# MakisChristou/fhestring

Measured on AMD Instinct MI355X. Metric: PBS/sec and ms/op for contains() on N-char FheString, higher is better.
Workload: dtype f64

## Files before the change

bindings/fhestring_hip.rs:

```rust
#![allow(non_camel_case_types, dead_code)]
use std::os::raw::{c_char, c_int, c_void};

pub const FHS_LWE_N: c_int = 742;
pub const FHS_POLY_N: c_int = 2048;
pub const FHS_BIG_CT: c_int = 2049;
pub const FHS_SMALL_CT: c_int = 743;
pub const FHS_BLOCKS_PER_CHAR: c_int = 4;
pub const FHS_CHAR_WORDS: usize = 8196;
pub const FHS_BSK_WORDS: usize = 6078464;
pub const FHS_KSK_WORDS: usize = 7608320;
pub const FHS_MAX_FIND_LENGTH: c_int = 255;
pub const FHS_MAX_REPETITIONS: c_int = 16;
pub const FHS_OK: c_int = 0;
pub const FHS_ERR_ARG: c_int = -1;
pub const FHS_ERR_HIP: c_int = -2;
pub const FHS_ERR_STATE: c_int = -3;
pub const FHS_ERR_LIMIT: c_int = -4;
pub const FHS_ARITH_EXACT_NTT: c_int = 0;
pub const FHS_ARITH_F64_FFT: c_int = 1;
pub const FHS_ARITH_F64_FFT_MB2: c_int = 2;
pub const FHS_ARITH_EXACT_NTT_MB2: c_int = 3;
pub const FHS_BSK_MB2_WORDS: usize = 9117696;
pub const FHS_MODE_AS_WRITTEN: c_int = 0;
pub const FHS_MODE_FUSED: c_int = 1;
pub const FHS_DIST_ID_BYTES: usize = 128;
pub const FHS_TRANSPORT_NONE: c_int = 0;
pub const FHS_TRANSPORT_RCCL: c_int = 1;
pub const FHS_TRANSPORT_HOST: c_int = 2;
pub const FHS_NOISE_BUDGET_SUM_C2: c_int = 64;
pub const FHS_DOM_SEEDED_STR: c_int = 4;
pub const FHS_DOM_SEEDED_BSK: c_int = 5;
pub const FHS_DOM_SEEDED_KSK: c_int = 6;
pub const FHS_SEED_WORDS: usize = 8;
pub const FHS_CSTR_BODY_WORDS: usize = 4;
pub const FHS_CBSK_BODY_WORDS: usize = 3039232;
pub const FHS_CKSK_BODY_WORDS: usize = 10240;
pub const FHS_CKEY_FILE_BYTES: usize = 24395872;
pub const FHS_PACK_BASE_LOG: c_int = 16;
pub const FHS_PACK_LEVELS: c_int = 3;
pub const FHS_PACK_TREE_LEVELS: c_int = 11;
pub const FHS_PACK_GROUP: c_int = 2048;
pub const FHS_PACK_KEY_WORDS: usize = 135168;
pub const FHS_PACK_KEY_FILE_BYTES: usize = 1081408;
// ... 147 lines not shown
    pub fn fhs_dist_str_compare(c: *mut fhs_ctx, a: *const fhs_char_t, na: usize, b: *const fhs_char_t, nb: usize, cmp: c_int, out: *mut fhs_char_t) -> c_int;
    pub fn fhs_dist_level_parallel(ctx: *mut fhs_ctx, on: c_int) -> c_int;
    pub fn fhs_dist_config(ctx: *mut fhs_ctx, rank: c_int, world: c_int) -> c_int;
    pub fn fhs_flush_plan(ctx: *mut fhs_ctx, n_levels: *mut u64, max_level_width: *mut u64) -> c_int;
    pub fn fhs_flush_level_exec(ctx: *mut fhs_ctx, level: u64, d_slice: *mut u64, width: *mut u64, cap: *mut u64) -> c_int;
    pub fn fhs_flush_level_commit(ctx: *mut fhs_ctx, level: u64, d_all: *const u64) -> c_int;
    pub fn fhs_stream_sync(ctx: *mut fhs_ctx) -> c_int;
    pub fn fhs_debug_capture_pbs_inputs(ctx: *mut fhs_ctx, max_rows_per_level: usize) -> c_int;
    pub fn fhs_debug_capture_live(ctx: *mut fhs_ctx, on: c_int) -> c_int;
    pub fn fhs_debug_capture_read(ctx: *mut fhs_ctx, rows: *mut u64, recs: *mut fhs_capture_rec, cap: usize, n: *mut usize) -> c_int;
    pub fn fhs_debug_plan_trace(ctx: *mut fhs_ctx, on: c_int) -> c_int;
    pub fn fhs_debug_plan_read(ctx: *mut fhs_ctx, out: *mut u64, cap: usize, n: *mut usize) -> c_int;
    pub fn fhs_debug_char_terms(ctx: *mut fhs_ctx, h: fhs_char_t, out: *mut u64, cap: usize, n: *mut usize) -> c_int;
    pub fn fhs_debug_lut_poly(lut_id: c_int, out: *mut u64) -> c_int;
    pub fn fhs_debug_live_resources(out: *mut u64) -> c_int;
    pub fn fhs_get_stats(ctx: *mut fhs_ctx, out: *mut fhs_stats) -> c_int;
    pub fn fhs_char_sum_c2(ctx: *mut fhs_ctx, h: fhs_char_t, out: *mut u64) -> c_int;
    pub fn fhs_char_set_noise(ctx: *mut fhs_ctx, h: fhs_char_t, sum_c2: u64) -> c_int;
    pub fn fhs_trivial_value(ctx: *mut fhs_ctx, h: fhs_char_t, is_trivial: *mut c_int, value: *mut u8) -> c_int;
    pub fn fhs_level_widths(ctx: *mut fhs_ctx, out: *mut u32, cap: usize, n: *mut usize) -> c_int;
    pub fn fhs_launch_groups(ctx: *mut fhs_ctx, out: *mut u32, cap: usize, n: *mut usize) -> c_int;
    pub fn fhs_reset_stats(ctx: *mut fhs_ctx) -> c_int;
    pub fn fhs_client_create(out: *mut *mut fhs_client) -> c_int;
    pub fn fhs_client_create_insecure_seeded(seed: u64, out: *mut *mut fhs_client) -> c_int;
    pub fn fhs_chacha20_block(key: *const u32, counter: u32, nonce: *const u32, out: *mut u32);
    pub fn fhs_chacha20_stream(key: *const u32, counter: u32, nonce: *const u32, out: *mut u64, n: usize);
    pub fn fhs_client_destroy(ck: *mut fhs_client);
    pub fn fhs_client_bsk(ck: *const fhs_client) -> *const u64;
    pub fn fhs_client_ksk(ck: *const fhs_client) -> *const u64;
    pub fn fhs_client_bsk_mb2(ck: *mut fhs_client) -> *const u64;
// ... 53 lines not shown
```

fhestring_amd/api.py:

```python
import ctypes as C

import numpy as np

from . import cabi
from ._lib import FhsError, lib, check_single_hip_runtime

_K = dict(cabi.parse_header()["consts"])
BIG_CT = _K["FHS_BIG_CT"]
SMALL_CT = _K["FHS_SMALL_CT"]
POLY_N = _K["FHS_POLY_N"]
PACK_GROUP = _K["FHS_PACK_GROUP"]
PACK_KEY_WORDS = _K["FHS_PACK_KEY_WORDS"]


def _ptr(a):
    return a.ctypes.data_as(C.c_void_p)


class Context:

    def __init__(self, device_id=0, planner=False):
        self._L = lib()
        if not planner:
            check_single_hip_runtime()
# ... 97 lines not shown
        return out

    def pbs_batch_shifted(self, cts, lut_idx, luts, shifts):
        cts = np.ascontiguousarray(cts, np.uint64).reshape(-1, BIG_CT)
        luts = np.ascontiguousarray(luts, np.uint64).reshape(-1, POLY_N)
        lut_idx = np.ascontiguousarray(lut_idx, np.uint32)
        B = cts.shape[0]
        shifts = np.ascontiguousarray(shifts, np.uint32).reshape(B, -1)
        out = np.zeros((B, shifts.shape[1], BIG_CT), np.uint64)
        self._check(self._L.fhs_pbs_batch_shifted(self._h, _ptr(cts), _ptr(lut_idx), _ptr(luts), luts.shape[0],
                                                  _ptr(shifts), shifts.shape[1], _ptr(out), B))
        return out

    def set_rotation_sharing(self, on=True):
        self._check(self._L.fhs_set_rotation_sharing(self._h, int(bool(on))))

    def keyswitch_modswitch_batch(self, cts):
        cts = np.ascontiguousarray(cts, np.uint64).reshape(-1, BIG_CT)
        B = cts.shape[0]
        out = np.zeros((B, SMALL_CT), np.uint32)
        self._check(self._L.fhs_keyswitch_modswitch_batch(self._h, _ptr(cts), _ptr(out), B))
        return out

    def pbs_batch_device(self, d_in, d_lut_idx, d_luts, d_out, B, stream=0):
        self._check(self._L.fhs_pbs_batch_device(self._h, C.c_void_p(d_in), C.c_void_p(d_lut_idx),
                                                 C.c_void_p(d_luts), C.c_void_p(d_out), int(B),
                                                 C.c_void_p(stream)))

    def kernel_timing(self, reset=False):
        br, ks = C.c_double(), C.c_double()
# ... 1046 lines not shown
```

fhestring_amd/csrc/capi_core.cpp:

```cpp
#include <algorithm>
#include <new>

#include "capi_internal.h"
#include "keyfile.h"
#include "luts.h"
#include "seeded_kernels.h"

extern "C" {

int fhs_ctx_create(int device_id, fhs_ctx **out) {
    if (!out) return FHS_ERR_ARG;
    *out = nullptr;
    fhs_ctx *c = new (std::nothrow) fhs_ctx();
    if (!c) return FHS_ERR_STATE;
    int rc = c->eng.ctx.init(device_id);
    if (rc) {
        *out = c;
        return rc;
    }
    *out = c;
    return FHS_OK;
}

int fhs_ctx_create_planner(fhs_ctx **out) {
// ... 187 lines not shown
    const fhs::Bid *b = ctx->eng.char_blocks(h);
    for (int k = 0; k < 4; k++) ctx->eng.describe_block(b[k], v);
    *n = v.size();
    if (!out) return FHS_OK;
    if (cap < v.size()) return ctx->eng.ctx.fail(FHS_ERR_ARG, "fhs_debug_char_terms: buffer too small");
    std::copy(v.begin(), v.end(), out);
    return FHS_OK;
}

int fhs_debug_live_resources(uint64_t out[5]) {
    if (!out) return FHS_ERR_ARG;
    fhs::live_resources(out);
    return FHS_OK;
}

int fhs_debug_lut_poly(int lut_id, uint64_t *out) {
    if (!out || lut_id < 0 || lut_id >= fhs::LUT_COUNT) return FHS_ERR_ARG;
    fhs::make_lut_poly(lut_id, out);
    return FHS_OK;
}

int fhs_debug_capture_read(fhs_ctx *ctx, uint64_t *rows, fhs_capture_rec *recs, size_t cap, size_t *n) {
    if (!ctx || !n) return FHS_ERR_ARG;
    auto &e = ctx->eng;
    static_assert(sizeof(fhs_capture_rec) == sizeof(fhs::Engine::CaptureRec), "record layout");
    const size_t have = e.capture_recs.size();
    if (!rows || !recs) { *n = have; return FHS_OK; }
    const size_t k = std::min(cap, have);
    std::copy(e.capture_rows.begin(), e.capture_rows.begin() + k * fhs::BIG_CT, rows);
    std::copy(e.capture_recs.begin(), e.capture_recs.begin() + k,
// ... 33 lines not shown
```

fhestring_amd/csrc/context.cpp:

```cpp
#include "context.h"
#include "pack_kernels.h"
#include "seeded_kernels.h"
#include "../../include/fhestring_hip.h"

#include <algorithm>
#include <cstdlib>
#include <utility>

namespace fhs {

namespace {
constexpr size_t KSK_BYTES = (size_t)BIG_N * KS_LEVEL * SMALL_CT * sizeof(uint64_t);
constexpr size_t BSK_BYTES = (size_t)LWE_N * 4 * POLY_N * sizeof(uint64_t);
}

#define HIP_TRY(expr, what)                                \
    do {                                                   \
        hipError_t e__ = (expr);                           \
        if (e__ != hipSuccess) return hip_fail(e__, what); \
    } while (0)

Event KernelTimer::get() {
    if (pool.empty()) return Event();
    Event e = std::move(pool.back());
// ... 60 lines not shown
            if (end == q) break;
            mask.push_back((uint32_t)w);
            bits += __builtin_popcount((uint32_t)w);
            q = *end == ',' ? end + 1 : end;
            if (*end != ',') break;
        }
        if (mask.empty() || bits == 0 || bits > cus) return fail(-1, "FHS_STREAM_CU_MASK: expected hex words selecting 1.." + std::to_string(cus) + " CUs");
        HIP_TRY(stream.create(mask.data(), (uint32_t)mask.size()), "hipExtStreamCreateWithCUMask");
        cus = bits;
    } else {
        HIP_TRY(stream.create(), "hipStreamCreate");
    }
    wg_slots = 4 * cus;
    launch_chunk[FHS_ARITH_F64_FFT_MB2] = (size_t)wg_slots;
    launch_chunk[FHS_ARITH_F64_FFT] = (size_t)wg_slots;
    HIP_TRY(d_work_counter.reserve_exact(64), "hipMalloc counter");
    return 0;
}

Context::~Context() {
    if (stream) (void)hipStreamSynchronize(stream);
    dist.shutdown();
    timer.resolve();
}

int Context::load_server_key(const uint64_t *bsk, const uint64_t *ksk) {
    if (!bsk || !ksk) return fail(-1, "null key pointer");
    HIP_TRY(hipSetDevice(device), "hipSetDevice");
    DevBuf d_ksk;
    HIP_TRY(d_ksk.reserve_exact(KSK_BYTES), "hipMalloc ksk staging");
    hipError_t e = hipMemcpy(d_ksk.ptr, ksk, KSK_BYTES, hipMemcpyHostToDevice);
// ... 108 lines not shown
}

int Context::keyswitch(const uint64_t *d_in, size_t B, hipStream_t s) {
    if (dig_buf.cap < ks_digits_bytes((int)B)) {
        HIP_TRY(hipStreamSynchronize(s), "sync");
        HIP_TRY(dig_buf.reserve(ks_digits_bytes((int)B)), "hipMalloc digits");
    }
    timer.begin(1, B, s);
    hipError_t e = launch_keyswitch_mfma(d_in, d_ksk_planes.as<int8_t>(), dig_buf.as<int8_t>(), ks_buf.as<uint64_t>(), (int)B, s,
                                         wg_slots / 4);
    timer.end(s);
    if (e != hipSuccess) return hip_fail(e, "keyswitch launch");
    return 0;
}

int Context::set_arithmetic(int mode) {
    if (mode < 0 || mode >= N_ARITH) return fail(-1, "unknown arithmetic mode");
    if (is_f64_fft(mode) && key_loaded && !d_bsk_fft)
        if (int rc = build_fft_key()) return rc;
    if (mode == FHS_ARITH_F64_FFT_MB2 && key_loaded && !d_bsk_mb)
        return fail(-3, "the two-bits-per-product arithmetic needs the pair key in the Fourier domain: call "
                        "fhs_load_multibit_key while arithmetic 1 (f64 FFT) is selected, then fhs_set_arithmetic 2");
    if (mode == FHS_ARITH_EXACT_NTT_MB2 && key_loaded && !d_bsk_ntt_mb)
        return fail(-3, "the exact two-bits-per-product arithmetic needs the pair key converted to residues: call "
                        "fhs_load_multibit_key while the EXACT arithmetic (fhs_set_arithmetic 0) is selected, then "
                        "fhs_set_arithmetic 3");
    arith = mode;
    return 0;
}

// ... 39 lines not shown
    HIP_TRY(prepare_device_for_packing(), "kernel attributes");
    return 0;
}

int Context::blind_rotate(const uint64_t *d_ks, const uint32_t *d_lut_idx, const uint64_t *d_luts, uint64_t *d_out,
                          uint64_t *const *d_out_ptrs, size_t B, hipStream_t s, uint64_t *const *d_body_ptrs) {
    hipError_t e = hipSuccess;
    const bool four = arith == FHS_ARITH_F64_FFT && B <= (size_t)fft4_max_batch;
    if (arith == FHS_ARITH_F64_FFT_MB2 && !d_bsk_mb) return fail(-3, "pair key not loaded (fhs_load_multibit_key)");
    if (arith == FHS_ARITH_EXACT_NTT_MB2 && !d_bsk_ntt_mb)
        return fail(-3, "pair key not loaded in the exact arithmetic (fhs_load_multibit_key)");
    if (arith == FHS_ARITH_F64_FFT && !d_bsk_fft) return fail(-3, "Fourier-domain key not loaded");
    timer.begin(four ? 2 : 0, B, s);
    const size_t chunk = (launch_chunk[arith] && !four) ? launch_chunk[arith] : B;
    uint32_t n_launches = 0;
    for (size_t off = 0, n = 0; off < B && e == hipSuccess; off += n) {
        n = std::min(chunk, B - off);
        if (B - off - n < chunk / 4) n = B - off;
        n_launches++;
        const uint64_t *ks = d_ks + off * SMALL_CT;
        const uint32_t *li = d_lut_idx + off;
        uint64_t *out = d_out ? d_out + off * BIG_CT : nullptr;
        uint64_t *const *outp = d_out_ptrs ? d_out_ptrs + off : nullptr;
        uint64_t *const *bodyp = d_body_ptrs ? d_body_ptrs + off : nullptr;
        if (arith == FHS_ARITH_EXACT_NTT_MB2) {
            BlindRotateNttMb2Params p{};
            p.ks = ks; p.lut_idx = li; p.luts = d_luts;
            p.bsk_ntt_mb = d_bsk_ntt_mb.as<double>(); p.tw = tw; p.crt_c = crt_c; p.mono = d_ntt_mono;
            p.out = out; p.out_ptrs = outp; p.body_ptrs = bodyp; p.B = (int)n;
            e = launch_blind_rotate_ntt_mb2(p, s);
        } else if (arith == FHS_ARITH_F64_FFT_MB2) {
            BlindRotateMb2Params p{};
            p.ks = ks; p.lut_idx = li; p.luts = d_luts;
            p.bsk_mb = d_bsk_mb.as<double>();
            p.lanetab = ft.lanetab; p.mono = ft.mono; p.r16 = ft.r16;
            p.work_counter = d_work_counter.as<uint32_t>();
            p.slots = wg_slots;
            p.out = out; p.out_ptrs = outp; p.body_ptrs = bodyp; p.B = (int)n;
            e = launch_blind_rotate_mb2(p, s);
        } else if (arith == FHS_ARITH_F64_FFT) {
            BlindRotateFftParams p{};
            p.ks = ks; p.lut_idx = li; p.luts = d_luts;
            p.bsk_fft = d_bsk_fft.as<double>();
            p.lanetab = ft.lanetab; p.weff = ft.weff;
            p.work_counter = d_work_counter.as<uint32_t>();
            p.slots = wg_slots;
            p.out = out; p.out_ptrs = outp; p.body_ptrs = bodyp; p.B = (int)n;
            e = four ? launch_blind_rotate_fft4(p, s) : launch_blind_rotate_fft(p, s);
        } else {
            BlindRotateParams p{};
            p.ks = ks; p.lut_idx = li; p.luts = d_luts;
            p.bsk_ntt = d_bsk_ntt.as<double>(); p.tw = tw; p.crt_c = crt_c;
            p.out = out; p.out_ptrs = outp; p.body_ptrs = bodyp; p.B = (int)n;
            e = launch_blind_rotate(p, s);
        }
    }
    timer.end(s, n_launches);
    if (e != hipSuccess) return hip_fail(e, "blind_rotate launch");
    return 0;
}

int Context::pbs_batch_device(const uint64_t *d_in, const uint32_t *d_lut_idx, const uint64_t *d_luts,
                              uint64_t *d_out, size_t B, hipStream_t s) {
// ... 117 lines not shown
```

fhestring_amd/csrc/context.h:

```cpp
#pragma once
#include <hip/hip_runtime.h>

#include <cstdint>
#include <string>
#include <vector>

#include "../../include/fhestring_hip.h"
#include "dist.h"
#include "fft_tables.h"
#include "hip_owners.h"
#include "ntt_tables.h"
#include "pbs_kernels.h"

namespace fhs {

constexpr int N_ARITH = 4;
constexpr bool is_f64_fft(int arith) { return arith == FHS_ARITH_F64_FFT || arith == FHS_ARITH_F64_FFT_MB2; }

struct FftTablePtrs {
    const double *lanetab = nullptr;
    const double *weff = nullptr;
    const double *mono = nullptr;
    const double *r16 = nullptr;
};
// ... 20 lines not shown
    std::string err;
    bool key_loaded = false;

    DevBuf d_ksk_planes;
    DevBuf d_bsk_ntt;
    DevBuf d_tables;
    NttTables tw{};
    double crt_c = 0;

    int arith = FHS_ARITH_EXACT_NTT;
    DevBuf d_bsk_fft;
    DevBuf d_bsk_std;
    DevBuf d_fft_tables;
    FftTablePtrs ft;
    DevBuf d_work_counter;
    int wg_slots = 1024;
    DevBuf d_bsk_mb;
    DevBuf d_bsk_ntt_mb;
    const double *d_ntt_mono = nullptr;
    DevBuf d_pack_key_ntt;
    int load_packing_key(const uint64_t *key);
    int load_multibit_key(const uint64_t *bsk_mb2);
    int fft4_max_batch = 512;
    size_t launch_chunk[N_ARITH] = {};
    int set_arithmetic(int mode);
    int keyswitch(const uint64_t *d_in, size_t B, hipStream_t s);
    int blind_rotate(const uint64_t *d_ks, const uint32_t *d_lut_idx, const uint64_t *d_luts, uint64_t *d_out,
                     uint64_t *const *d_out_ptrs, size_t B, hipStream_t s, uint64_t *const *d_body_ptrs = nullptr);

    Dist dist;
    DevBuf xchg_send, xchg_recv;

    DevBuf dig_buf;
    DevBuf ks_buf, ms_buf, in_buf, out_buf, lutidx_buf, luts_buf, tab_buf;
    DevBuf pack_ws[2], pack_tab, pack_out;
    KernelTimer timer;

    int init(int device_id);
    ~Context();
    int fail(int code, const std::string &msg) { err = msg; return code; }
    int hip_fail(hipError_t e, const char *what);
// ... 18 lines not shown
```

fhestring_amd/csrc/engine.cpp:

```cpp
#include "engine.h"
#include "../../include/fhestring_hip.h"

#include <algorithm>
#include <cstdio>
#include <cstdlib>
#include <cstring>
#include <map>

namespace fhs {

int Engine::on_key_loaded() {
    if (!d_luts_) {
        std::vector<uint64_t> host((size_t)LUT_COUNT * POLY_N);
        for (int id = 0; id < LUT_COUNT; id++) make_lut_poly(id, host.data() + (size_t)id * POLY_N);
        hipError_t e = d_luts_.reserve_exact(host.size() * 8);
        if (e != hipSuccess) return ctx.hip_fail(e, "hipMalloc luts");
        e = hipMemcpy(d_luts_.ptr, host.data(), host.size() * 8, hipMemcpyHostToDevice);
        if (e != hipSuccess) return ctx.hip_fail(e, "copy luts");
    }
    return 0;
}

Engine::~Engine() {
    if (!planner && ctx.stream) (void)hipStreamSynchronize(ctx.stream);
// ... 714 lines not shown
        CaptureRec r = l.recs[first + i];
        r.level = level;
        capture_recs.push_back(r);
    }
    return 0;
}

int Engine::launch_rows(const GroupView &v, size_t lo, size_t cnt, uint64_t *dense_out, const TickLevel *levels,
                        size_t n_levels, size_t first_level) {
    const uint8_t *dp = tick_buf_.as<uint8_t>();
    const LinDesc *d_desc = reinterpret_cast<const LinDesc *>(dp);
    const LinTerm *d_terms = reinterpret_cast<const LinTerm *>(dp + v.off_terms);
    const uint32_t *d_lut = reinterpret_cast<const uint32_t *>(dp + v.off_lut);
    uint64_t *const *d_out = reinterpret_cast<uint64_t *const *>(dp + v.off_out);
    uint64_t *const *d_body = reinterpret_cast<uint64_t *const *>(dp + v.off_body);
    hipError_t e = launch_lincomb(d_desc + lo, d_terms, batch_in_.as<uint64_t>(), (int)cnt, ctx.stream);
    if (e != hipSuccess) return ctx.hip_fail(e, "lincomb launch");
    size_t row0 = 0;
    for (size_t j = 0; j < n_levels && capture_max_rows; j++) {
        const TickLevel &l = levels[j];
        const size_t w = l.descs.size(), a = std::max(lo, row0), b = std::min(lo + cnt, row0 + w);
        if (l.recs.size() == w && a < b)
            if (int rc = sample_capture(l, a - row0, b - a, a - lo, (uint32_t)(first_level + j))) return rc;
        row0 += w;
    }
    if (int rc = ctx.keyswitch(batch_in_.as<uint64_t>(), cnt, ctx.stream)) return rc;
    return ctx.blind_rotate(ctx.ks_buf.as<uint64_t>(), d_lut + lo, d_luts_.as<uint64_t>(), dense_out, dense_out ? nullptr : d_out + lo, cnt,
                            ctx.stream, v.n_ext && !dense_out ? d_body + lo : nullptr);
}

int Engine::scatter_rows(const uint64_t *d_all, uint64_t *const *d_out, size_t width) {
    hipError_t e = launch_scatter_blocks(d_all, d_out, (int)width, ctx.stream);
    return e == hipSuccess ? 0 : ctx.hip_fail(e, "scatter launch");
}

void Engine::trace_group(const std::vector<TickLevel> &levels, size_t width) {
    for (auto &l : levels) {
        for (size_t k = 0; k < l.descs.size(); k++) {
            const LinDesc &d = l.descs[k];
            trace_.insert(trace_.end(), {TR_ROW, (uint64_t)(uintptr_t)l.out[k], l.lut[k], d.konst_body >> DELTA_LOG, d.n_terms});
            for (uint32_t t = 0; t < d.n_terms; t++) {
// ... 177 lines not shown
```

fhestring_amd/csrc/ks_kernels.hip:

```cpp
#include <cstdlib>

#include "pbs_kernels.h"

namespace fhs {

namespace {
typedef int v4i __attribute__((ext_vector_type(4)));
typedef int v16i __attribute__((ext_vector_type(16)));

constexpr int KS_K = BIG_N * KS_LEVEL;
constexpr int KS_STEPS = KS_K / 32;
constexpr int KS_COL_TILES = 24;
constexpr int KS_PLANES = 8;

__device__ __forceinline__ size_t frag_off(int r, int k) {
    return ((size_t)(k >> 5) * 64 + ((k >> 4) & 1) * 32 + r) * 16 + (k & 15);
}
}

__global__ __launch_bounds__(256) void ks_digits_kernel(const uint64_t *__restrict__ in, int8_t *__restrict__ dig, int B) {
    const int ct = blockIdx.x;
    int8_t *dst = dig + (size_t)(ct >> 5) * KS_STEPS * 1024;
    const int r = ct & 31;
    for (int i = threadIdx.x; i < BIG_N; i += 256) {
// ... 45 lines not shown
                    d[l] = x;
                }
            }
#pragma unroll
            for (int l = 0; l < KS_LEVEL; l++) {
                const int p = pos + l;
                if (p >= 0 && p < 16) w[p >> 2] |= (uint32_t)(uint8_t)(int8_t)d[l] << (8 * (p & 3));
            }
        }
        v4i o;
        o.x = (int)w[0]; o.y = (int)w[1]; o.z = (int)w[2]; o.w = (int)w[3];
        dst[(size_t)ks * 64] = o;
    }
}

__global__ __launch_bounds__(256) void ksk_to_planes_kernel(const uint64_t *__restrict__ ksk, int8_t *__restrict__ planes) {
    const int k = blockIdx.x;
    for (int j = threadIdx.x; j < KS_COL_TILES * 32; j += 256) {
        uint64_t w = j < SMALL_CT ? ksk[(size_t)k * SMALL_CT + j] : 0;
        const size_t off = (size_t)(j >> 5) * KS_STEPS * 1024 + frag_off(j & 31, k);
#pragma unroll
        for (int b = 0; b < KS_PLANES; b++) {
            const int8_t s = (int8_t)(w & 0xff);
            w = (w - (uint64_t)(int64_t)s) >> 8;
            planes[(size_t)b * KS_COL_TILES * KS_STEPS * 1024 + off] = s;
        }
    }
}

__global__ __launch_bounds__(256) void keyswitch_mfma_kernel(const int8_t *__restrict__ dig, const int8_t *__restrict__ planes,
// ... 147 lines not shown
}

hipError_t prepare_device_for_keyswitch() {
    return hipFuncSetAttribute(reinterpret_cast<const void *>(keyswitch_mfma2_kernel),
                               hipFuncAttributeMaxDynamicSharedMemorySize, KS2_LDS_BYTES);
}

size_t ks_planes_bytes() { return (size_t)KS_PLANES * KS_COL_TILES * KS_STEPS * 1024; }
size_t ks_digits_bytes(int B) { return (size_t)((B + 255) / 256) * 8 * KS_STEPS * 1024; }

hipError_t launch_ksk_to_planes(const uint64_t *d_ksk, int8_t *d_planes, hipStream_t s) {
    hipLaunchKernelGGL(ksk_to_planes_kernel, dim3(KS_K), dim3(256), 0, s, d_ksk, d_planes);
    return hipGetLastError();
}

hipError_t launch_keyswitch_mfma(const uint64_t *d_in, const int8_t *d_planes, int8_t *d_dig, uint64_t *d_ks_out, int B,
                                 hipStream_t s, int n_cus) {
    if (B <= 0) return hipSuccess;
    const int tiles = (B + 31) / 32;
    static const int old_below = [] { const char *v = std::getenv("FHS_KS_OLD_BELOW"); return v ? std::atoi(v) : KS2_MIN_BATCH; }();
    const bool wide = B >= old_below;
    if (wide)
        hipLaunchKernelGGL(ks_digits_tile_kernel, dim3(((B + KS2_GROUP - 1) / KS2_GROUP) * (KS2_GROUP / 32), KS_DIG_CHUNKS),
                           dim3(256), 0, s, d_in, d_dig, B);
    else
        hipLaunchKernelGGL(ks_digits_kernel, dim3(((tiles + 3) / 4) * 128), dim3(256), 0, s, d_in, d_dig, B);
    hipError_t e = hipGetLastError();
    if (e != hipSuccess) return e;
    if (wide) {
        const int n_groups = (B + KS2_GROUP - 1) / KS2_GROUP;
        const int tiles2 = KS_COL_TILES * n_groups, slots = n_cus > 0 ? n_cus : 256;
        int full = tiles2 / slots * slots, rem = tiles2 - full, slices = 1;
        if (rem > 0)
            for (int c : {8, 4, 2})
                if (rem * c <= slots) { slices = c; break; }
        if (slices == 1) { full = tiles2; rem = 0; }
        else {
            const size_t row0 = (size_t)(full / 8 / 3) * KS2_GROUP;
            if (row0 < (size_t)B) {
                e = hipMemsetAsync(d_ks_out + row0 * SMALL_CT, 0, ((size_t)B - row0) * SMALL_CT * 8, s);
                if (e != hipSuccess) return e;
            }
        }
        hipLaunchKernelGGL(keyswitch_mfma2_kernel, dim3(full + rem * slices), dim3(256), KS2_LDS_BYTES, s, d_dig, d_planes,
                           d_in, d_ks_out, B, n_groups, full, rem > 0 ? rem : 1, slices);
        return hipGetLastError();
    }
    int splits = 1;
    const int tgroups = (tiles + 3) / 4;
    while (splits < 16 && tgroups * KS_COL_TILES * splits < 256) splits *= 2;
    if (splits > 1) {
        e = hipMemsetAsync(d_ks_out, 0, (size_t)B * SMALL_CT * 8, s);
        if (e != hipSuccess) return e;
    }
    hipLaunchKernelGGL(keyswitch_mfma_kernel, dim3(tgroups, KS_COL_TILES, splits), dim3(256), 0, s, d_dig, d_planes,
                       d_in, d_ks_out, B, KS_STEPS / splits);
    return hipGetLastError();
}

}
```

fhestring_amd/csrc/pbs_kernels.h:

```cpp
#pragma once
#include <hip/hip_runtime.h>
#include <cstddef>
#include <cstdint>

namespace fhs {

constexpr int LWE_N = 742;
constexpr int POLY_N = 2048;
constexpr int BIG_N = 2048;
constexpr int BIG_CT = 2049;
constexpr int SMALL_CT = 743;
constexpr int KS_LEVEL = 5;
constexpr int KS_BASE_LOG = 3;
constexpr int DELTA_LOG = 59;
constexpr int BSK_QUANT_BITS = 6;

constexpr uint64_t NTT_P0 = 140737488273409ull;
constexpr uint64_t NTT_P1 = 140737488252929ull;
constexpr uint64_t NTT_PSI0 = 124135596386681ull;
constexpr uint64_t NTT_PSI1 = 116052249937262ull;

struct NttTables {
    const double *fwd_uni;
    const double *fwd_lane;
// ... 62 lines not shown
struct LinDesc {
    uint32_t first_term;
    uint32_t n_terms;
    uint64_t konst_body;
};
struct LinTerm {
    const uint64_t *src;
    int64_t coef;
};

size_t blind_rotate_lds_bytes();
hipError_t prepare_device_for_kernels();
hipError_t read_device_ntt_consts(double *fwd_uni , double *inv_uni , double *crt);
hipError_t launch_blind_rotate(const BlindRotateParams &p, hipStream_t s);
hipError_t launch_blind_rotate_fft(const BlindRotateFftParams &p, hipStream_t s);
hipError_t launch_blind_rotate_fft4(const BlindRotateFftParams &p, hipStream_t s);
hipError_t launch_bsk_to_fft(const uint64_t *d_bsk_std, double *d_out, const double *d_lanetab, hipStream_t s,
                             int n_polys = LWE_N * 4);
hipError_t launch_blind_rotate_mb2(const BlindRotateMb2Params &p, hipStream_t s);
hipError_t launch_blind_rotate_ntt_mb2(const BlindRotateNttMb2Params &p, hipStream_t s);
hipError_t prepare_device_for_ntt_mb2();
hipError_t prepare_device_for_fft4();
hipError_t prepare_device_for_keyswitch();
void fft_uniform_consts(double *w_re, double *w_im, double *u_re, double *u_im);
size_t ks_planes_bytes();
size_t ks_digits_bytes(int B);
hipError_t launch_ksk_to_planes(const uint64_t *d_ksk, int8_t *d_planes, hipStream_t s);
hipError_t launch_keyswitch_mfma(const uint64_t *d_in , const int8_t *d_planes, int8_t *d_dig ,
                                 uint64_t *d_ks_out , int B, hipStream_t s, int n_cus = 256);
hipError_t launch_modswitch(const uint64_t *d_ks, uint32_t *d_ms , int B, hipStream_t s);
hipError_t launch_lincomb(const LinDesc *d_desc, const LinTerm *d_terms, uint64_t *d_out ,
                          int n, hipStream_t s);
hipError_t launch_scatter_blocks(const uint64_t *d_in, uint64_t *const *d_dst, int n, hipStream_t s);
hipError_t launch_gather_rows(const uint64_t *const *d_src, uint64_t *d_out, int n, hipStream_t s);
struct ExtractDesc {
    const uint64_t *lead;
    const uint64_t *body;
    uint64_t *out;
    uint32_t K, pad;
};
hipError_t launch_extract_shift(const ExtractDesc *d_desc, int n, hipStream_t s);

}
```

include/fhestring_hip.h:

```cpp
#ifndef FHESTRING_HIP_H
#define FHESTRING_HIP_H

#include <stddef.h>
#include <stdint.h>

#ifdef __cplusplus
extern "C" {
#endif

#define FHS_LWE_N 742
#define FHS_POLY_N 2048
#define FHS_BIG_CT 2049
#define FHS_SMALL_CT 743
#define FHS_BLOCKS_PER_CHAR 4
#define FHS_CHAR_WORDS (4 * 2049)
#define FHS_BSK_WORDS ((size_t)742 * 4 * 2048)
#define FHS_KSK_WORDS ((size_t)2048 * 5 * 743)
#define FHS_MAX_FIND_LENGTH 255
#define FHS_MAX_REPETITIONS 16

#define FHS_OK 0
#define FHS_ERR_ARG (-1)
#define FHS_ERR_HIP (-2)
#define FHS_ERR_STATE (-3)
// ... 151 lines not shown
    uint32_t lut;
    uint32_t n_terms;
    int64_t sum_c2;
    int32_t konst;
    uint32_t width;
} fhs_capture_rec;
int fhs_debug_capture_pbs_inputs(fhs_ctx *ctx, size_t max_rows_per_level);
int fhs_debug_capture_live(fhs_ctx *ctx, int on);
int fhs_debug_capture_read(fhs_ctx *ctx, uint64_t *rows, fhs_capture_rec *recs, size_t cap, size_t *n);

int fhs_debug_plan_trace(fhs_ctx *ctx, int on);
int fhs_debug_plan_read(fhs_ctx *ctx, uint64_t *out, size_t cap, size_t *n);
int fhs_debug_char_terms(fhs_ctx *ctx, fhs_char_t h, uint64_t *out, size_t cap, size_t *n);
int fhs_debug_lut_poly(int lut_id, uint64_t *out);
int fhs_debug_live_resources(uint64_t out[5]);

typedef struct {
    uint64_t pbs_executed;
    uint64_t pbs_folded;
    uint64_t levels;
    uint64_t max_level_width;
    uint64_t blocks_live;
    uint64_t max_input_sum_c2;
    uint64_t pbs_shared;
    uint64_t pbs_extracted;
} fhs_stats;
#define FHS_NOISE_BUDGET_SUM_C2 64
int fhs_get_stats(fhs_ctx *ctx, fhs_stats *out);
int fhs_char_sum_c2(fhs_ctx *ctx, fhs_char_t h, uint64_t *out);
int fhs_char_set_noise(fhs_ctx *ctx, fhs_char_t h, uint64_t sum_c2);
// ... 106 lines not shown
```

Baseline: 138,300.

## Fuse lincomb with keyswitch digit extraction and rotate work counters in a ring

Adds a fused kernel that computes the linear combination and, in the same pass, decomposes it into keyswitch digits and clears the keyswitch output. The keyswitch then runs only the MFMA product stage, which removes a separate digits kernel, a memset and a re-read of the lincomb output. It also keeps a ring of 1024 device work counters so each FFT blind-rotate launch gets a fresh zeroed counter, with one bulk memset per ring wrap instead of per-launch resets. Both paths are on by default and can be switched off through a new debug flag API.

```diff
diff --git a/bindings/fhestring_hip.rs b/bindings/fhestring_hip.rs
--- a/bindings/fhestring_hip.rs
+++ b/bindings/fhestring_hip.rs
@@ -27,6 +27,9 @@
 pub const FHS_TRANSPORT_NONE: c_int = 0;
 pub const FHS_TRANSPORT_RCCL: c_int = 1;
 pub const FHS_TRANSPORT_HOST: c_int = 2;
+pub const FHS_GROUP_FUSED_DIGITS: c_int = 1;
+pub const FHS_GROUP_COUNTER_RING: c_int = 2;
+pub const FHS_GROUP_ALL: c_int = 3;
 pub const FHS_NOISE_BUDGET_SUM_C2: c_int = 64;
 pub const FHS_DOM_SEEDED_STR: c_int = 4;
 pub const FHS_DOM_SEEDED_BSK: c_int = 5;
@@ -204,6 +207,9 @@
     pub fn fhs_debug_char_terms(ctx: *mut fhs_ctx, h: fhs_char_t, out: *mut u64, cap: usize, n: *mut usize) -> c_int;
     pub fn fhs_debug_lut_poly(lut_id: c_int, out: *mut u64) -> c_int;
     pub fn fhs_debug_live_resources(out: *mut u64) -> c_int;
+    pub fn fhs_debug_set_group_paths(ctx: *mut fhs_ctx, flags: u32) -> c_int;
+    pub fn fhs_debug_digits_bytes(n_rows: usize) -> usize;
+    pub fn fhs_debug_lincomb_keyswitch(ctx: *mut fhs_ctx, src: *const u64, n_src: usize, n_terms: *const u32, konst_body: *const u64, term_src: *const u32, term_coef: *const i64, n_rows: usize, rows_out: *mut u64, digits_out: *mut c_void, ks_out: *mut u64) -> c_int;
     pub fn fhs_get_stats(ctx: *mut fhs_ctx, out: *mut fhs_stats) -> c_int;
     pub fn fhs_char_sum_c2(ctx: *mut fhs_ctx, h: fhs_char_t, out: *mut u64) -> c_int;
     pub fn fhs_char_set_noise(ctx: *mut fhs_ctx, h: fhs_char_t, sum_c2: u64) -> c_int;
diff --git a/fhestring_amd/api.py b/fhestring_amd/api.py
--- a/fhestring_amd/api.py
+++ b/fhestring_amd/api.py
@@ -135,6 +135,28 @@
 
     def set_rotation_sharing(self, on=True):
         self._check(self._L.fhs_set_rotation_sharing(self._h, int(bool(on))))
+
+    GROUP_FUSED_DIGITS = _K["FHS_GROUP_FUSED_DIGITS"]
+    GROUP_COUNTER_RING = _K["FHS_GROUP_COUNTER_RING"]
+    GROUP_ALL = _K["FHS_GROUP_ALL"]
+
+    def set_group_paths(self, flags):
+        self._check(self._L.fhs_debug_set_group_paths(self._h, int(flags)))
+
+    def lincomb_keyswitch(self, src, n_terms, konst_body, term_src, term_coef):
+        src = np.ascontiguousarray(src, np.uint64).reshape(-1, BIG_CT)
+        n_terms = np.ascontiguousarray(n_terms, np.uint32)
+        konst_body = np.ascontiguousarray(konst_body, np.uint64)
+        term_src = np.ascontiguousarray(term_src, np.uint32)
+        term_coef = np.ascontiguousarray(term_coef, np.int64)
+        B = n_terms.size
+        assert konst_body.size == B and term_src.size == term_coef.size == int(n_terms.sum())
+        rows = np.zeros((B, BIG_CT), np.uint64)
+        dig = np.zeros(self._L.fhs_debug_digits_bytes(B), np.int8)
+        ks = np.zeros((B, SMALL_CT), np.uint64)
+        self._check(self._L.fhs_debug_lincomb_keyswitch(self._h, _ptr(src), src.shape[0], _ptr(n_terms), _ptr(konst_body),
+                                                        _ptr(term_src), _ptr(term_coef), B, _ptr(rows), _ptr(dig), _ptr(ks)))
+        return rows, dig, ks
 
     def keyswitch_modswitch_batch(self, cts):
         cts = np.ascontiguousarray(cts, np.uint64).reshape(-1, BIG_CT)
diff --git a/fhestring_amd/csrc/capi_core.cpp b/fhestring_amd/csrc/capi_core.cpp
--- a/fhestring_amd/csrc/capi_core.cpp
+++ b/fhestring_amd/csrc/capi_core.cpp
@@ -225,6 +225,26 @@
     return FHS_OK;
 }
 
+int fhs_debug_set_group_paths(fhs_ctx *ctx, uint32_t flags) {
+    if (!ctx) return FHS_ERR_ARG;
+    if (flags & ~(uint32_t)FHS_GROUP_ALL) return ctx->eng.ctx.fail(FHS_ERR_ARG, "fhs_debug_set_group_paths: unknown flag");
+    if (int rc = ctx->eng.flush()) return rc;
+    ctx->eng.ctx.group_paths = flags;
+    return FHS_OK;
+}
+
+size_t fhs_debug_digits_bytes(size_t n_rows) { return fhs::ks_digits_bytes((int)n_rows); }
+
+int fhs_debug_lincomb_keyswitch(fhs_ctx *ctx, const uint64_t *src, size_t n_src, const uint32_t *n_terms,
+                                const uint64_t *konst_body, const uint32_t *term_src, const int64_t *term_coef, size_t n_rows,
+                                uint64_t *rows_out, void *digits_out, uint64_t *ks_out) {
+    if (!ctx) return FHS_ERR_ARG;
+    if (ctx->eng.planner) return ctx->eng.ctx.fail(FHS_ERR_STATE, "planner context: nothing is computed");
+    if (int rc = ctx->eng.flush()) return rc;
+    return ctx->eng.ctx.lincomb_keyswitch_host(src, n_src, n_terms, konst_body, term_src, term_coef, n_rows, rows_out, digits_out,
+                                               ks_out);
+}
+
 int fhs_debug_lut_poly(int lut_id, uint64_t *out) {
     if (!out || lut_id < 0 || lut_id >= fhs::LUT_COUNT) return FHS_ERR_ARG;
     fhs::make_lut_poly(lut_id, out);
diff --git a/fhestring_amd/csrc/context.cpp b/fhestring_amd/csrc/context.cpp
--- a/fhestring_amd/csrc/context.cpp
+++ b/fhestring_amd/csrc/context.cpp
@@ -98,7 +98,8 @@
     wg_slots = 4 * cus;
     launch_chunk[FHS_ARITH_F64_FFT_MB2] = (size_t)wg_slots;
     launch_chunk[FHS_ARITH_F64_FFT] = (size_t)wg_slots;
-    HIP_TRY(d_work_counter.reserve_exact(64), "hipMalloc counter");
+    HIP_TRY(d_work_counter.reserve_exact((WORK_COUNTERS + 1) * sizeof(uint32_t)), "hipMalloc counters");
+    HIP_TRY(hipMemset(d_work_counter.ptr, 0, (WORK_COUNTERS + 1) * sizeof(uint32_t)), "clear counters");
     return 0;
 }
 
@@ -237,6 +238,72 @@
     return 0;
 }
 
+int Context::lincomb_digits(const LinDesc *d_desc, const LinTerm *d_terms, uint64_t *d_out, size_t B, hipStream_t s) {
+    if (dig_buf.cap < ks_digits_bytes((int)B)) {
+        HIP_TRY(hipStreamSynchronize(s), "sync");
+        HIP_TRY(dig_buf.reserve(ks_digits_bytes((int)B)), "hipMalloc digits");
+    }
+    hipError_t e = launch_lincomb_digits(d_desc, d_terms, d_out, dig_buf.as<int8_t>(), ks_buf.as<uint64_t>(), (int)B, s, wg_slots / 4);
+    if (e != hipSuccess) return hip_fail(e, "lincomb launch");
+    return 0;
+}
+
+int Context::keyswitch_product(const uint64_t *d_in, size_t B, hipStream_t s) {
+    timer.begin(1, B, s);
+    hipError_t e = launch_keyswitch_product(d_in, d_ksk_planes.as<int8_t>(), dig_buf.as<int8_t>(), ks_buf.as<uint64_t>(), (int)B, s,
+                                            wg_slots / 4);
+    timer.end(s);
+    if (e != hipSuccess) return hip_fail(e, "keyswitch launch");
+    return 0;
+}
+
+int Context::lincomb_keyswitch_host(const uint64_t *src, size_t n_src, const uint32_t *n_terms, const uint64_t *konst_body,
+                                    const uint32_t *term_src, const int64_t *term_coef, size_t B, uint64_t *batch_in,
+                                    void *digits, uint64_t *ks_out) {
+    if (!key_loaded) return fail(-3, "server key not loaded");
+    if (!src || !n_terms || !konst_body || !term_src || !term_coef || !batch_in || !digits || !ks_out) return fail(-1, "null pointer");
+    if (B == 0 || B > (size_t)1 << 16 || n_src == 0) return fail(-1, "row or source count out of range");
+    HIP_TRY(hipSetDevice(device), "hipSetDevice");
+    std::vector<LinDesc> descs(B);
+    size_t total = 0;
+    for (size_t r = 0; r < B; r++) {
+        descs[r] = LinDesc{(uint32_t)total, n_terms[r], konst_body[r]};
+        total += n_terms[r];
+    }
+    HIP_TRY(in_buf.reserve(n_src * BIG_CT * 8), "hipMalloc");
+    HIP_TRY(out_buf.reserve(B * BIG_CT * 8), "hipMalloc");
+    std::vector<LinTerm> terms(total);
+    for (size_t t = 0; t < total; t++) {
+        if (term_src[t] >= n_src) return fail(-1, "term source out of range");
+        terms[t] = LinTerm{in_buf.as<uint64_t>() + (size_t)term_src[t] * BIG_CT, term_coef[t]};
+    }
+    const size_t desc_bytes = B * sizeof(LinDesc), dig_bytes = ks_digits_bytes((int)B);
+    HIP_TRY(tab_buf.reserve(desc_bytes + std::max<size_t>(total, 1) * sizeof(LinTerm)), "hipMalloc");
+    HIP_TRY(ks_buf.reserve(B * SMALL_CT * 8), "hipMalloc ks");
+    HIP_TRY(hipStreamSynchronize(stream), "sync");
+    HIP_TRY(dig_buf.reserve(dig_bytes), "hipMalloc digits");
+    const LinDesc *d_desc = tab_buf.as<LinDesc>();
+    const LinTerm *d_terms = reinterpret_cast<const LinTerm *>(tab_buf.as<uint8_t>() + desc_bytes);
+    HIP_TRY(hipMemcpy(in_buf.ptr, src, n_src * BIG_CT * 8, hipMemcpyHostToDevice), "H2D");
+    HIP_TRY(hipMemcpy(tab_buf.ptr, descs.data(), desc_bytes, hipMemcpyHostToDevice), "H2D");
+    if (total) HIP_TRY(hipMemcpy(tab_buf.as<uint8_t>() + desc_bytes, terms.data(), total * sizeof(LinTerm), hipMemcpyHostToDevice), "H2D");
+    HIP_TRY(hipMemset(dig_buf.ptr, 0x55, dig_bytes), "fill");
+    HIP_TRY(hipMemset(ks_buf.ptr, 0xFF, B * SMALL_CT * 8), "fill");
+    HIP_TRY(hipMemset(out_buf.ptr, 0xFF, B * BIG_CT * 8), "fill");
+    if (group_paths & FHS_GROUP_FUSED_DIGITS) {
+        if (int rc = lincomb_digits(d_desc, d_terms, out_buf.as<uint64_t>(), B, stream)) return rc;
+        if (int rc = keyswitch_product(out_buf.as<uint64_t>(), B, stream)) return rc;
+    } else {
+        HIP_TRY(launch_lincomb(d_desc, d_terms, out_buf.as<uint64_t>(), (int)B, stream), "lincomb launch");
+        if (int rc = keyswitch(out_buf.as<uint64_t>(), B, stream)) return rc;
+    }
+    HIP_TRY(hipStreamSynchronize(stream), "sync");
+    HIP_TRY(hipMemcpy(batch_in, out_buf.ptr, B * BIG_CT * 8, hipMemcpyDeviceToHost), "D2H");
+    HIP_TRY(hipMemcpy(digits, dig_buf.ptr, dig_bytes, hipMemcpyDeviceToHost), "D2H");
+    HIP_TRY(hipMemcpy(ks_out, ks_buf.ptr, B * SMALL_CT * 8, hipMemcpyDeviceToHost), "D2H");
+    return 0;
+}
+
 int Context::set_arithmetic(int mode) {
     if (mode < 0 || mode >= N_ARITH) return fail(-1, "unknown arithmetic mode");
     if (is_f64_fft(mode) && key_loaded && !d_bsk_fft)
@@ -306,6 +373,13 @@
     timer.begin(four ? 2 : 0, B, s);
     const size_t chunk = (launch_chunk[arith] && !four) ? launch_chunk[arith] : B;
     uint32_t n_launches = 0;
+    const bool ring = (group_paths & FHS_GROUP_COUNTER_RING) != 0;
+    auto take_work_counter = [&] { return d_work_counter.as<uint32_t>() + (ring ? work_counter_next : WORK_COUNTERS); };
+    auto counter_taken = [&] {
+        if (!ring || ++work_counter_next < WORK_COUNTERS) return hipSuccess;
+        work_counter_next = 0;
+        return hipMemsetAsync(d_work_counter.ptr, 0, WORK_COUNTERS * sizeof(uint32_t), s);
+    };
     for (size_t off = 0, n = 0; off < B && e == hipSuccess; off += n) {
         n = std::min(chunk, B - off);
         if (B - off - n < chunk / 4) n = B - off;
@@ -326,7 +400,7 @@
             p.ks = ks; p.lut_idx = li; p.luts = d_luts;
             p.bsk_mb = d_bsk_mb.as<double>();
             p.lanetab = ft.lanetab; p.mono = ft.mono; p.r16 = ft.r16;
-            p.work_counter = d_work_counter.as<uint32_t>();
+            p.work_counter = d_work_counter.as<uint32_t>() + WORK_COUNTERS;
             p.slots = wg_slots;
             p.out = out; p.out_ptrs = outp; p.body_ptrs = bodyp; p.B = (int)n;
             e = launch_blind_rotate_mb2(p, s);
@@ -335,10 +409,14 @@
             p.ks = ks; p.lut_idx = li; p.luts = d_luts;
             p.bsk_fft = d_bsk_fft.as<double>();
             p.lanetab = ft.lanetab; p.weff = ft.weff;
-            p.work_counter = d_work_counter.as<uint32_t>();
             p.slots = wg_slots;
             p.out = out; p.out_ptrs = outp; p.body_ptrs = bodyp; p.B = (int)n;
-            e = four ? launch_blind_rotate_fft4(p, s) : launch_blind_rotate_fft(p, s);
+            if (four) e = launch_blind_rotate_fft4(p, s);
+            else {
+                p.work_counter = take_work_counter();
+                e = ring ? launch_blind_rotate_fft_fresh_counter(p, s) : launch_blind_rotate_fft(p, s);
+                if (e == hipSuccess) e = counter_taken();
+            }
         } else {
             BlindRotateParams p{};
             p.ks = ks; p.lut_idx = li; p.luts = d_luts;
diff --git a/fhestring_amd/csrc/context.h b/fhestring_amd/csrc/context.h
--- a/fhestring_amd/csrc/context.h
+++ b/fhestring_amd/csrc/context.h
@@ -58,6 +58,9 @@
     DevBuf d_fft_tables;
     FftTablePtrs ft;
     DevBuf d_work_counter;
+    static constexpr uint32_t WORK_COUNTERS = 1024;
+    uint32_t work_counter_next = 0;
+    uint32_t group_paths = FHS_GROUP_ALL;
     int wg_slots = 1024;
     DevBuf d_bsk_mb;
     DevBuf d_bsk_ntt_mb;
@@ -69,6 +72,11 @@
     size_t launch_chunk[N_ARITH] = {};
     int set_arithmetic(int mode);
     int keyswitch(const uint64_t *d_in, size_t B, hipStream_t s);
+    int lincomb_digits(const LinDesc *d_desc, const LinTerm *d_terms, uint64_t *d_out, size_t B, hipStream_t s);
+    int keyswitch_product(const uint64_t *d_in, size_t B, hipStream_t s);
+    int lincomb_keyswitch_host(const uint64_t *src, size_t n_src, const uint32_t *n_terms, const uint64_t *konst_body,
+                               const uint32_t *term_src, const int64_t *term_coef, size_t B, uint64_t *batch_in, void *digits,
+                               uint64_t *ks_out);
     int blind_rotate(const uint64_t *d_ks, const uint32_t *d_lut_idx, const uint64_t *d_luts, uint64_t *d_out,
                      uint64_t *const *d_out_ptrs, size_t B, hipStream_t s, uint64_t *const *d_body_ptrs = nullptr);
 
diff --git a/fhestring_amd/csrc/engine.cpp b/fhestring_amd/csrc/engine.cpp
--- a/fhestring_amd/csrc/engine.cpp
+++ b/fhestring_amd/csrc/engine.cpp
@@ -752,8 +752,13 @@
     const uint32_t *d_lut = reinterpret_cast<const uint32_t *>(dp + v.off_lut);
     uint64_t *const *d_out = reinterpret_cast<uint64_t *const *>(dp + v.off_out);
     uint64_t *const *d_body = reinterpret_cast<uint64_t *const *>(dp + v.off_body);
-    hipError_t e = launch_lincomb(d_desc + lo, d_terms, batch_in_.as<uint64_t>(), (int)cnt, ctx.stream);
-    if (e != hipSuccess) return ctx.hip_fail(e, "lincomb launch");
+    const bool fused = (ctx.group_paths & FHS_GROUP_FUSED_DIGITS) != 0;
+    if (fused) {
+        if (int rc = ctx.lincomb_digits(d_desc + lo, d_terms, batch_in_.as<uint64_t>(), cnt, ctx.stream)) return rc;
+    } else {
+        hipError_t e = launch_lincomb(d_desc + lo, d_terms, batch_in_.as<uint64_t>(), (int)cnt, ctx.stream);
+        if (e != hipSuccess) return ctx.hip_fail(e, "lincomb launch");
+    }
     size_t row0 = 0;
     for (size_t j = 0; j < n_levels && capture_max_rows; j++) {
         const TickLevel &l = levels[j];
@@ -762,7 +767,9 @@
             if (int rc = sample_capture(l, a - row0, b - a, a - lo, (uint32_t)(first_level + j))) return rc;
         row0 += w;
     }
-    if (int rc = ctx.keyswitch(batch_in_.as<uint64_t>(), cnt, ctx.stream)) return rc;
+    if (int rc = fused ? ctx.keyswitch_product(batch_in_.as<uint64_t>(), cnt, ctx.stream)
+                       : ctx.keyswitch(batch_in_.as<uint64_t>(), cnt, ctx.stream))
+        return rc;
     return ctx.blind_rotate(ctx.ks_buf.as<uint64_t>(), d_lut + lo, d_luts_.as<uint64_t>(), dense_out, dense_out ? nullptr : d_out + lo, cnt,
                             ctx.stream, v.n_ext && !dense_out ? d_body + lo : nullptr);
 }
diff --git a/fhestring_amd/csrc/ks_kernels.hip b/fhestring_amd/csrc/ks_kernels.hip
--- a/fhestring_amd/csrc/ks_kernels.hip
+++ b/fhestring_amd/csrc/ks_kernels.hip
@@ -83,6 +83,89 @@
     }
 }
 
+constexpr int LD_COEFS = BIG_N / KS_DIG_CHUNKS;
+constexpr int LD_STRIDE = LD_COEFS + 2;
+static_assert(LD_COEFS * KS_LEVEL == (KS_STEPS / KS_DIG_CHUNKS) * 32, "a chunk of coefficients is a whole number of k-steps");
+__global__ __launch_bounds__(256) void lincomb_digits_kernel(const LinDesc *__restrict__ desc, const LinTerm *__restrict__ terms,
+                                                             uint64_t *__restrict__ out, int8_t *__restrict__ dig,
+                                                             uint64_t *__restrict__ ks_out, int B, int clear_from) {
+    __shared__ uint16_t v15[32 * LD_STRIDE];
+    const int tile = blockIdx.x, chunk = blockIdx.y;
+    const int lane = threadIdx.x & 63, wave = threadIdx.x >> 6;
+    const int e0 = chunk * LD_COEFS;
+    for (int rr = wave; rr < 32; rr += 4) {
+        const int ct = tile * 32 + rr;
+        uint64_t v[4] = {0, 0, 0, 0};
+        if (ct < B) {
+            const LinDesc d = desc[ct];
+            for (uint32_t t = 0; t < d.n_terms; t++) {
+                const LinTerm tm = terms[d.first_term + t];
+#pragma unroll
+                for (int q = 0; q < 4; q++) v[q] += (uint64_t)tm.coef * tm.src[e0 + lane + 64 * q];
+            }
+            uint64_t *o = out + (size_t)ct * BIG_CT + e0;
+#pragma unroll
+            for (int q = 0; q < 4; q++) o[lane + 64 * q] = v[q];
+        }
+#pragma unroll
+        for (int q = 0; q < 4; q++)
+            v15[rr * LD_STRIDE + lane + 64 * q] = (uint16_t)((v[q] + (1ull << 48)) >> 49);
+    }
+    if (chunk == 0 && threadIdx.x < 32) {
+        const int ct = tile * 32 + (int)threadIdx.x;
+        if (ct < B) {
+            const LinDesc d = desc[ct];
+            uint64_t v = d.konst_body;
+            for (uint32_t t = 0; t < d.n_terms; t++) {
+                const LinTerm tm = terms[d.first_term + t];
+                v += (uint64_t)tm.coef * tm.src[BIG_N];
+            }
+            out[(size_t)ct * BIG_CT + BIG_N] = v;
+        }
+    }
+    {
+        constexpr int COLS = (SMALL_CT + KS_DIG_CHUNKS - 1) / KS_DIG_CHUNKS;
+        const int c0 = chunk * COLS, c1 = c0 + COLS < SMALL_CT ? c0 + COLS : SMALL_CT;
+        const int r0 = tile * 32 > clear_from ? tile * 32 : clear_from, r1 = tile * 32 + 32 < B ? tile * 32 + 32 : B;
+        const int w = c1 - c0;
+        for (int x = threadIdx.x; x < (r1 - r0) * w; x += 256) ks_out[(size_t)(r0 + x / w) * SMALL_CT + c0 + x % w] = 0;
+    }
+    __syncthreads();
+    const int r = lane & 31, h = lane >> 5;
+    const uint16_t *row = v15 + r * LD_STRIDE;
+    v4i *dst = reinterpret_cast<v4i *>(dig + (size_t)tile * KS_STEPS * 1024) + lane;
+    const int ks_begin = chunk * (KS_STEPS / KS_DIG_CHUNKS), ks_end = ks_begin + KS_STEPS / KS_DIG_CHUNKS;
+    for (int ks = ks_begin + wave; ks < ks_end; ks += 4) {
+        const int k0 = ks * 32 + h * 16;
+        const int i0 = k0 / KS_LEVEL, l0 = k0 - i0 * KS_LEVEL;
+        uint32_t w[4] = {0, 0, 0, 0};
+        int pos = -l0;
+#pragma unroll
+        for (int c = 0; c < 4; c++, pos += KS_LEVEL) {
+            const int il = i0 + c - e0;
+            int d[KS_LEVEL] = {0, 0, 0, 0, 0};
+            if (il < LD_COEFS) {
+                uint32_t v = row[il];
+#pragma unroll
+                for (int l = KS_LEVEL - 1; l >= 0; l--) {
+                    int x = (int)(v & 7u);
+                    v >>= 3;
+                    if (x >= 4) { x -= 8; v += 1; }
+                    d[l] = x;
+                }
+            }
+#pragma unroll
+            for (int l = 0; l < KS_LEVEL; l++) {
+                const int p = pos + l;
+                if (p >= 0 && p < 16) w[p >> 2] |= (uint32_t)(uint8_t)(int8_t)d[l] << (8 * (p & 3));
+            }
+        }
+        v4i o;
+        o.x = (int)w[0]; o.y = (int)w[1]; o.z = (int)w[2]; o.w = (int)w[3];
+        dst[(size_t)ks * 64] = o;
+    }
+}
+
 __global__ __launch_bounds__(256) void ksk_to_planes_kernel(const uint64_t *__restrict__ ksk, int8_t *__restrict__ planes) {
     const int k = blockIdx.x;
     for (int j = threadIdx.x; j < KS_COL_TILES * 32; j += 256) {
@@ -260,48 +343,83 @@
     return hipGetLastError();
 }
 
+namespace {
+struct KsShape {
+    bool wide;
+    int tiles_padded;
+    int n_groups, full, rem, slices;
+    int tgroups, splits;
+    int clear_from;
+};
+KsShape ks_shape(int B, int n_cus) {
+    KsShape k{};
+    const int tiles = (B + 31) / 32;
+    static const int old_below = [] { const char *v = std::getenv("FHS_KS_OLD_BELOW"); return v ? std::atoi(v) : KS2_MIN_BATCH; }();
+    k.wide = B >= old_below;
+    k.clear_from = B;
+    if (k.wide) {
+        k.n_groups = (B + KS2_GROUP - 1) / KS2_GROUP;
+        k.tiles_padded = k.n_groups * (KS2_GROUP / 32);
+        const int tiles2 = KS_COL_TILES * k.n_groups, slots = n_cus > 0 ? n_cus : 256;
+        k.full = tiles2 / slots * slots; k.rem = tiles2 - k.full; k.slices = 1;
+        if (k.rem > 0)
+            for (int c : {8, 4, 2})
+                if (k.rem * c <= slots) { k.slices = c; break; }
+        if (k.slices == 1) { k.full = tiles2; k.rem = 0; }
+        else {
+            const int row0 = (k.full / 8 / 3) * KS2_GROUP;
+            if (row0 < B) k.clear_from = row0;
+        }
+        return k;
+    }
+    k.tgroups = (tiles + 3) / 4;
+    k.tiles_padded = k.tgroups * 4;
+    k.splits = 1;
+    while (k.splits < 16 && k.tgroups * KS_COL_TILES * k.splits < 256) k.splits *= 2;
+    if (k.splits > 1) k.clear_from = 0;
+    return k;
+}
+hipError_t launch_ks_product(const KsShape &k, const uint64_t *d_in, const int8_t *d_planes, const int8_t *d_dig,
+                             uint64_t *d_ks_out, int B, hipStream_t s) {
+    if (k.wide)
+        hipLaunchKernelGGL(keyswitch_mfma2_kernel, dim3(k.full + k.rem * k.slices), dim3(256), KS2_LDS_BYTES, s, d_dig, d_planes,
+                           d_in, d_ks_out, B, k.n_groups, k.full, k.rem > 0 ? k.rem : 1, k.slices);
+    else
+        hipLaunchKernelGGL(keyswitch_mfma_kernel, dim3(k.tgroups, KS_COL_TILES, k.splits), dim3(256), 0, s, d_dig, d_planes,
+                           d_in, d_ks_out, B, KS_STEPS / k.splits);
+    return hipGetLastError();
+}
+}
+
 hipError_t launch_keyswitch_mfma(const uint64_t *d_in, const int8_t *d_planes, int8_t *d_dig, uint64_t *d_ks_out, int B,
                                  hipStream_t s, int n_cus) {
     if (B <= 0) return hipSuccess;
-    const int tiles = (B + 31) / 32;
-    static const int old_below = [] { const char *v = std::getenv("FHS_KS_OLD_BELOW"); return v ? std::atoi(v) : KS2_MIN_BATCH; }();
-    const bool wide = B >= old_below;
-    if (wide)
-        hipLaunchKernelGGL(ks_digits_tile_kernel, dim3(((B + KS2_GROUP - 1) / KS2_GROUP) * (KS2_GROUP / 32), KS_DIG_CHUNKS),
-                           dim3(256), 0, s, d_in, d_dig, B);
+    const KsShape k = ks_shape(B, n_cus);
+    if (k.wide)
+        hipLaunchKernelGGL(ks_digits_tile_kernel, dim3(k.tiles_padded, KS_DIG_CHUNKS), dim3(256), 0, s, d_in, d_dig, B);
     else
-        hipLaunchKernelGGL(ks_digits_kernel, dim3(((tiles + 3) / 4) * 128), dim3(256), 0, s, d_in, d_dig, B);
+        hipLaunchKernelGGL(ks_digits_kernel, dim3(k.tiles_padded * 32), dim3(256), 0, s, d_in, d_dig, B);
     hipError_t e = hipGetLastError();
     if (e != hipSuccess) return e;
-    if (wide) {
-        const int n_groups = (B + KS2_GROUP - 1) / KS2_GROUP;
-        const int tiles2 = KS_COL_TILES * n_groups, slots = n_cus > 0 ? n_cus : 256;
-        int full = tiles2 / slots * slots, rem = tiles2 - full, slices = 1;
-        if (rem > 0)
-            for (int c : {8, 4, 2})
-                if (rem * c <= slots) { slices = c; break; }
-        if (slices == 1) { full = tiles2; rem = 0; }
-        else {
-            const size_t row0 = (size_t)(full / 8 / 3) * KS2_GROUP;
-            if (row0 < (size_t)B) {
-                e = hipMemsetAsync(d_ks_out + row0 * SMALL_CT, 0, ((size_t)B - row0) * SMALL_CT * 8, s);
-                if (e != hipSuccess) return e;
-            }
-        }
-        hipLaunchKernelGGL(keyswitch_mfma2_kernel, dim3(full + rem * slices), dim3(256), KS2_LDS_BYTES, s, d_dig, d_planes,
-                           d_in, d_ks_out, B, n_groups, full, rem > 0 ? rem : 1, slices);
-        return hipGetLastError();
-    }
-    int splits = 1;
-    const int tgroups = (tiles + 3) / 4;
-    while (splits < 16 && tgroups * KS_COL_TILES * splits < 256) splits *= 2;
-    if (splits > 1) {
-        e = hipMemsetAsync(d_ks_out, 0, (size_t)B * SMALL_CT * 8, s);
+    if (k.clear_from < B) {
+        e = hipMemsetAsync(d_ks_out + (size_t)k.clear_from * SMALL_CT, 0, (size_t)(B - k.clear_from) * SMALL_CT * 8, s);
         if (e != hipSuccess) return e;
     }
-    hipLaunchKernelGGL(keyswitch_mfma_kernel, dim3(tgroups, KS_COL_TILES, splits), dim3(256), 0, s, d_dig, d_planes,
-                       d_in, d_ks_out, B, KS_STEPS / splits);
+    return launch_ks_product(k, d_in, d_planes, d_dig, d_ks_out, B, s);
+}
+
+hipError_t launch_lincomb_digits(const LinDesc *d_desc, const LinTerm *d_terms, uint64_t *d_out, int8_t *d_dig,
+                                 uint64_t *d_ks_out, int B, hipStream_t s, int n_cus) {
+    if (B <= 0) return hipSuccess;
+    const KsShape k = ks_shape(B, n_cus);
+    hipLaunchKernelGGL(lincomb_digits_kernel, dim3(k.tiles_padded, KS_DIG_CHUNKS), dim3(256), 0, s, d_desc, d_terms, d_out,
+                       d_dig, d_ks_out, B, k.clear_from);
     return hipGetLastError();
 }
-
-}
+hipError_t launch_keyswitch_product(const uint64_t *d_in, const int8_t *d_planes, const int8_t *d_dig, uint64_t *d_ks_out,
+                                    int B, hipStream_t s, int n_cus) {
+    if (B <= 0) return hipSuccess;
+    return launch_ks_product(ks_shape(B, n_cus), d_in, d_planes, d_dig, d_ks_out, B, s);
+}
+
+}
diff --git a/fhestring_amd/csrc/pbs_kernels.h b/fhestring_amd/csrc/pbs_kernels.h
--- a/fhestring_amd/csrc/pbs_kernels.h
+++ b/fhestring_amd/csrc/pbs_kernels.h
@@ -100,6 +100,7 @@
 hipError_t read_device_ntt_consts(double *fwd_uni , double *inv_uni , double *crt);
 hipError_t launch_blind_rotate(const BlindRotateParams &p, hipStream_t s);
 hipError_t launch_blind_rotate_fft(const BlindRotateFftParams &p, hipStream_t s);
+hipError_t launch_blind_rotate_fft_fresh_counter(const BlindRotateFftParams &p, hipStream_t s);
 hipError_t launch_blind_rotate_fft4(const BlindRotateFftParams &p, hipStream_t s);
 hipError_t launch_bsk_to_fft(const uint64_t *d_bsk_std, double *d_out, const double *d_lanetab, hipStream_t s,
                              int n_polys = LWE_N * 4);
@@ -114,6 +115,10 @@
 hipError_t launch_ksk_to_planes(const uint64_t *d_ksk, int8_t *d_planes, hipStream_t s);
 hipError_t launch_keyswitch_mfma(const uint64_t *d_in , const int8_t *d_planes, int8_t *d_dig ,
                                  uint64_t *d_ks_out , int B, hipStream_t s, int n_cus = 256);
+hipError_t launch_lincomb_digits(const LinDesc *d_desc, const LinTerm *d_terms, uint64_t *d_out , int8_t *d_dig,
+                                 uint64_t *d_ks_out , int B, hipStream_t s, int n_cus = 256);
+hipError_t launch_keyswitch_product(const uint64_t *d_in , const int8_t *d_planes, const int8_t *d_dig,
+                                    uint64_t *d_ks_out , int B, hipStream_t s, int n_cus = 256);
 hipError_t launch_modswitch(const uint64_t *d_ks, uint32_t *d_ms , int B, hipStream_t s);
 hipError_t launch_lincomb(const LinDesc *d_desc, const LinTerm *d_terms, uint64_t *d_out ,
                           int n, hipStream_t s);
diff --git a/fhestring_amd/csrc/rotate_launch.hip b/fhestring_amd/csrc/rotate_launch.hip
--- /dev/null
+++ b/fhestring_amd/csrc/rotate_launch.hip
@@ -0,0 +1,16 @@
+#include "fft_device.h"
+#include "pbs_kernels.h"
+
+namespace fhs {
+
+__global__ __launch_bounds__(128, 2) void blind_rotate_fft_kernel(BlindRotateFftParams P);
+
+hipError_t launch_blind_rotate_fft_fresh_counter(const BlindRotateFftParams &p, hipStream_t s) {
+    if (p.B <= 0) return hipSuccess;
+    const size_t lds = (size_t)2 * fftdev::FFT_LDS_DOUBLES * sizeof(double) + 16;
+    const int grid = p.B < p.slots ? p.B : p.slots;
+    hipLaunchKernelGGL(blind_rotate_fft_kernel, dim3(grid), dim3(128), lds, s, p);
+    return hipGetLastError();
+}
+
+}
diff --git a/include/fhestring_hip.h b/include/fhestring_hip.h
--- a/include/fhestring_hip.h
+++ b/include/fhestring_hip.h
@@ -189,6 +189,14 @@
 int fhs_debug_char_terms(fhs_ctx *ctx, fhs_char_t h, uint64_t *out, size_t cap, size_t *n);
 int fhs_debug_lut_poly(int lut_id, uint64_t *out);
 int fhs_debug_live_resources(uint64_t out[5]);
+#define FHS_GROUP_FUSED_DIGITS 1
+#define FHS_GROUP_COUNTER_RING 2
+#define FHS_GROUP_ALL 3
+int fhs_debug_set_group_paths(fhs_ctx *ctx, uint32_t flags);
+size_t fhs_debug_digits_bytes(size_t n_rows);
+int fhs_debug_lincomb_keyswitch(fhs_ctx *ctx, const uint64_t *src , size_t n_src, const uint32_t *n_terms,
+                                const uint64_t *konst_body, const uint32_t *term_src, const int64_t *term_coef, size_t n_rows,
+                                uint64_t *rows_out, void *digits_out, uint64_t *ks_out);
 
 typedef struct {
     uint64_t pbs_executed;
```

Measured after the change: 138,300, median of 2. Within noise of the previous version (-0.0%).
